# peaceminusones/Group-GAN-GCN-GAT

Hardware: AMD Instinct MI355X
Metric: scenes/sec (obs8/pred12, 20 peds) at 1/2/4/8 GPUs; ADE/FDE vs ref (higher is better)
Workload: dtype fp32; 1 GPU; train iteration = D-step + G-step (best_k=20, Adam), GAT generator; BASELINE configs[1] shape (batch 64); scenes_per_gpu=64, global_batch=64, obs_len=8, pred_len=12, generator=gat, hip_graph=True, parallelism=dp1

## Files before the change

### group-gan-gcn-gat_amd/csrc/glue.hip

```cpp
#include "sgg_common.h"

namespace sgg {

namespace {

__global__ void __launch_bounds__(256) traj_cat_kernel(const float* __restrict__ head, int ldh, int T0,
                                                       const float* __restrict__ a, int lda,
                                                       const float* __restrict__ b, int ldb, int T1, int B,
                                                       float* __restrict__ out, const float* __restrict__ pos0,
                                                       float* __restrict__ start) {
  const int NB = b ? 2 * B : B;
  const int total = (T0 + T1) * NB;
  for (int e = blockIdx.x * blockDim.x + threadIdx.x; e < total + (start ? NB : 0); e += gridDim.x * blockDim.x) {
    if (e >= total) {
      const int p = e - total;
      reinterpret_cast<float2*>(start)[p] = reinterpret_cast<const float2*>(pos0)[p < B ? p : p - B];
      continue;
    }
    const int t = e / NB, p = e - t * NB;
    const float* src;
    if (t < T0) {
      src = head + (size_t)t * ldh + 2 * (p < B ? p : p - B);
    } else if (p < B) {
      src = a + (size_t)(t - T0) * lda + 2 * p;
// ... 8 lines not shown
                                                           const float* __restrict__ z, int nz,
                                                           const int64_t* __restrict__ best, int first_k,
                                                           int copies, const int32_t* __restrict__ ped_scene,
                                                           int S, int B, const float* __restrict__ last_rel,
                                                           float* __restrict__ h0, float* __restrict__ rel0) {
  const int D = Dc + nz;
  const int total = copies * B * D;
  for (int e = blockIdx.x * blockDim.x + threadIdx.x; e < total; e += gridDim.x * blockDim.x) {
    const int row = e / D, c = e - row * D;
    const int r = row / B, p = row - r * B;
    float v;
    if (c < Dc) {
      v = ctx[(size_t)p * ldc + c];
    } else {
      const int s = ped_scene[p];
      const int k = (best && r == 0) ? (int)best[s] : first_k + r - (best ? 1 : 0);
      v = z[((size_t)k * S + s) * nz + (c - Dc)];
    }
    h0[e] = v;
    if (c < 2) rel0[(size_t)row * 2 + c] = last_rel[(size_t)p * 2 + c];
  }
}

constexpr int kL2MaxElems = SGG_POOL_MAX_PEDS * 32;

__device__ __forceinline__ void stage_mask(float* msk, const float* __restrict__ mask, int ldm, int o, int n, int T,
                                           int t0, int nt) {
  for (int e = t0; e < n * T; e += nt) {
    const int i = e / T, t = e - i * T;
    msk[e] = mask[(size_t)(o + i) * ldm + t];
  }
}

__global__ void __launch_bounds__(512) l2_select_kernel(const float* __restrict__ pred, const float* __restrict__ gt,
                                                        const float* __restrict__ mask, int ldm,
                                                        const int32_t* __restrict__ scene_off, int T, int B, int k,
                                                        int64_t* __restrict__ best) {
  __shared__ float part[256];
  __shared__ float msk[kL2MaxElems];
  const int s = blockIdx.x;
  const int o = scene_off[s], n = scene_off[s + 1] - o;
  const int lane = threadIdx.x & 63, wave = threadIdx.x >> 6;
  const float2* g2 = reinterpret_cast<const float2*>(gt);
  const float2* p2 = reinterpret_cast<const float2*>(pred);
  const int tot = n * T;
  const bool staged = tot <= kL2MaxElems;
  if (staged) stage_mask(msk, mask, ldm, o, n, T, threadIdx.x, blockDim.x);
  __syncthreads();
  constexpr int kRS = 4;
  for (int r0 = wave; r0 < k; r0 += 8 * kRS) {
    float acc[kRS];
#pragma unroll
    for (int j = 0; j < kRS; ++j) acc[j] = 0.f;
    for (int e0 = lane; e0 < tot; e0 += 256) {
      float mk[4];
      float2 g[4], q[kRS][4];
#pragma unroll
      for (int u = 0; u < 4; ++u) {
        const int e = min(e0 + 64 * u, tot - 1);
        const int t = e / n, i = e - t * n, p = o + i;
        mk[u] = staged ? msk[i * T + t] : mask[(size_t)p * ldm + t];
        g[u] = g2[(size_t)t * B + p];
#pragma unroll
        for (int j = 0; j < kRS; ++j) {
          const int r = min(r0 + 8 * j, k - 1);
          q[j][u] = p2[((size_t)t * k + r) * B + p];
        }
      }
#pragma unroll
      for (int j = 0; j < kRS; ++j)
#pragma unroll
        for (int u = 0; u < 4; ++u)
          if (e0 + 64 * u < tot) {
            const float dx = g[u].x - q[j][u].x, dy = g[u].y - q[j][u].y;
            acc[j] = fmaf(mk[u], fmaf(dx, dx, dy * dy), acc[j]);
          }
    }
#pragma unroll
    for (int j = 0; j < kRS; ++j) {
      const float a = wave_sum(acc[j]);
      if (lane == 0 && r0 + 8 * j < k) part[r0 + 8 * j] = a;
    }
  }
  __syncthreads();
  if (threadIdx.x == 0) {
    int bi = 0;
    float bv = part[0];
    for (int r = 1; r < k; ++r)
      if (part[r] < bv) {
        bv = part[r];
        bi = r;
      }
    best[s] = bi;
  }
}

__device__ __forceinline__ void l2_scene(const float* __restrict__ pred, int ldp, const float2* __restrict__ g2,
                                         const float* __restrict__ mask, int ldm, int o, int n, int T, int B,
                                         float* msk, int lane, float& acc_out, float& ms_out) {
  const int tot = n * T;
  const bool staged = tot <= kL2MaxElems;
  if (staged) stage_mask(msk, mask, ldm, o, n, T, lane, 64);
  __builtin_amdgcn_fence(__ATOMIC_RELEASE, "wavefront");
  __builtin_amdgcn_wave_barrier();
  __builtin_amdgcn_fence(__ATOMIC_ACQUIRE, "wavefront");
  float acc = 0.f, ms = 0.f;
  for (int e0 = lane; e0 < tot; e0 += 256) {
    float mk[4];
    float2 g[4], q[4];
#pragma unroll
    for (int u = 0; u < 4; ++u) {
      const int e = min(e0 + 64 * u, tot - 1);
      const int t = e / n, i = e - t * n, p = o + i;
      mk[u] = staged ? msk[i * T + t] : mask[(size_t)p * ldm + t];
      g[u] = g2[(size_t)t * B + p];
      q[u] = *reinterpret_cast<const float2*>(pred + (size_t)t * ldp + 2 * p);
    }
// ... 99 lines not shown
  hipLaunchKernelGGL(traj_cat_kernel, dim3(grid_for(total, 256)), dim3(256), 0, (hipStream_t)stream, head, ldh, T0, a,
                     lda, b, ldb, T1, B, out, pos0, start);
  SGG_RETURN_LAUNCH("sgg_traj_cat");
}

extern "C" int sgg_decoder_init(const float* ctx, int ldc, int Dc, const float* z, int nz, const int64_t* best,
                                int first_k, int copies, const int32_t* ped_scene, int S, int B,
                                const float* last_rel, float* h0, float* rel0, void* stream) {
  SGG_CHECK_ARG(ctx && ped_scene && last_rel && h0 && rel0 && (nz == 0 || z), "sgg_decoder_init: null pointer");
  SGG_CHECK_ARG(Dc > 0 && nz >= 0 && ldc >= Dc && copies >= 1 && S >= 0 && B >= 0 && Dc + nz >= 2,
                "sgg_decoder_init: bad sizes");
  const long long total = (long long)copies * B * (Dc + nz);
  if (total == 0) return 0;
  hipLaunchKernelGGL(decoder_init_kernel, dim3(grid_for(total, 256)), dim3(256), 0, (hipStream_t)stream, ctx, ldc, Dc,
                     z, nz, best, first_k, copies, ped_scene, S, B, last_rel, h0, rel0);
  SGG_RETURN_LAUNCH("sgg_decoder_init");
}

extern "C" int sgg_l2_select(const float* pred, const float* gt, const float* mask, int ldm, const int32_t* scene_off,
                             int S, int T, int B, int k, int64_t* best, void* stream) {
  SGG_CHECK_ARG(pred && gt && mask && scene_off && best, "sgg_l2_select: null pointer");
  SGG_CHECK_ARG(S >= 0 && T >= 1 && B >= 0 && k >= 1 && k <= 256 && ldm >= T, "sgg_l2_select: bad sizes");
  if (S == 0) return 0;
  hipLaunchKernelGGL(l2_select_kernel, dim3(S), dim3(512), 0, (hipStream_t)stream, pred, gt, mask, ldm, scene_off, T,
                     B, k, best);
  SGG_RETURN_LAUNCH("sgg_l2_select");
}

extern "C" int sgg_l2_loss_fwd(const float* pred, int ldp, const float* gt, const float* mask, int ldm,
                               const int32_t* scene_off, int S, int T, int B, float w, float* loss, float* msum,
                               float* term_ws, void* stream) {
  SGG_CHECK_ARG(pred && gt && mask && scene_off && loss && msum && term_ws, "sgg_l2_loss_fwd: null pointer");
  SGG_CHECK_ARG(S >= 0 && T >= 1 && B >= 0 && ldm >= T && ldp >= 2 * B, "sgg_l2_loss_fwd: bad sizes");
  if (S > 0)
    hipLaunchKernelGGL(l2_terms_kernel, dim3(S), dim3(64), 0, (hipStream_t)stream, pred, ldp, gt, mask, ldm, scene_off,
                     T, B, w, msum, term_ws);
  hipLaunchKernelGGL(l2_sum_kernel, dim3(1), dim3(64), 0, (hipStream_t)stream, term_ws, S, loss);
  SGG_RETURN_LAUNCH("sgg_l2_loss_fwd");
}

extern "C" int sgg_l2_loss_bwd(const float* pred, int ldp, const float* gt, const float* mask, int ldm,
                               const int32_t* ped_scene, const float* msum, int T, int B, float w, const float* gout,
                               float* dpred, int ldd, void* stream) {
  SGG_CHECK_ARG(pred && gt && mask && ped_scene && msum && gout && dpred, "sgg_l2_loss_bwd: null pointer");
  SGG_CHECK_ARG(T >= 1 && B >= 0 && ldm >= T && ldp >= 2 * B && ldd >= 2 * B, "sgg_l2_loss_bwd: bad sizes");
  if (B == 0) return 0;
  hipLaunchKernelGGL(l2_loss_bwd_kernel, dim3(grid_for((long long)T * B, 256)), dim3(256), 0, (hipStream_t)stream,
                     pred, ldp, gt, mask, ldm, ped_scene, msum, T, B, w, gout, dpred, ldd);
// ... 15 lines not shown
```

### group-gan-gcn-gat_amd/csrc/grad.hip

```cpp
#include <string.h>

#include "sgg_common.h"

namespace sgg {

namespace {

constexpr int kRedJobs = SGG_RED_MAX + 2 * SGG_FOLDB_MAX;

struct FinishArgs {
  SggRed red[kRedJobs];
  unsigned char vec[kRedJobs];
  int nred;
  int blk0[kRedJobs + 1];
  SggL2Job l2[SGG_LOSSJOB_MAX];
  SggBceJob bce[SGG_LOSSJOB_MAX];
  int nl2, nbce;
};

__device__ __forceinline__ float phase_sum(const float* __restrict__ src, int rows, int ld, int col, int ph) {
  float s = 0.f;
  int r = ph;
  for (; r + 48 < rows; r += 64) {
    const float v0 = src[(size_t)r * ld + col], v1 = src[(size_t)(r + 16) * ld + col];
    const float v2 = src[(size_t)(r + 32) * ld + col], v3 = src[(size_t)(r + 48) * ld + col];
    s += v0;
    s += v1;
    s += v2;
    s += v3;
  }
  for (; r < rows; r += 16) s += src[(size_t)r * ld + col];
  return s;
}

__device__ __forceinline__ floatx4 phase_sum4(const float* __restrict__ src, int rows, int ld, int col, int ph) {
  floatx4 s = {0.f, 0.f, 0.f, 0.f};
  int r = ph;
  for (; r + 48 < rows; r += 64) {
    const floatx4 v0 = *reinterpret_cast<const floatx4*>(src + (size_t)r * ld + col);
    const floatx4 v1 = *reinterpret_cast<const floatx4*>(src + (size_t)(r + 16) * ld + col);
// ... 130 lines not shown
  for (int j = 0; j < SGG_LOSSJOB_MAX; ++j)
    if (j < a.nbce) bce_load(a.bce[j], in[j]);
  float ad[SGG_LOSSJOB_MAX];
#pragma unroll
  for (int j = 0; j < SGG_LOSSJOB_MAX; ++j) {
    ad[j] = 0.f;
    if (j < a.nbce && a.bce[j].total) {
      bool fromL2 = false;
      for (int k = 0; k < a.nl2; ++k) fromL2 |= a.bce[j].addend == a.l2[k].loss;
      if (!fromL2) ad[j] = *a.bce[j].addend;
    }
  }
  for (int k = 0; k < a.nl2; ++k) l2_value(a.l2[k], lv + k);
#pragma unroll
  for (int j = 0; j < SGG_LOSSJOB_MAX; ++j)
    if (j < a.nbce) {
      float addend = ad[j];
      for (int k = 0; k < a.nl2; ++k)
        if (a.bce[j].total && a.bce[j].addend == a.l2[k].loss) addend = lv[k];
      bce_value(a.bce[j], in[j], addend, reinterpret_cast<float(*)[kLossThreads / 64]>(&rpart[0][0]));
    }
}

__global__ void __launch_bounds__(1024) grad_finish_kernel(FinishArgs a) {
  __shared__ __attribute__((aligned(16))) float rpart[16][256];
  const int lw = a.nl2 + a.nbce > 0;
  const int b = (int)blockIdx.x - lw;
  if (b < 0) {
    loss_workgroup(a, rpart);
    return;
  }
  int j = 0;
  while (j + 1 < a.nred && b >= a.blk0[j + 1]) ++j;
  red_job(a.red[j], a.vec[j] != 0, b - a.blk0[j], rpart);
}

}

}

using namespace sgg;

extern "C" int sgg_grad_finish(const SggRed* reds, int nred, const SggFoldBwd* folds, int nfold, float* scratch,
                               size_t scratch_bytes, void* stream) {
  return sgg_grad_finish_losses(reds, nred, folds, nfold, scratch, scratch_bytes, nullptr, 0, nullptr, 0, stream);
}

extern "C" int sgg_grad_finish_losses(const SggRed* reds, int nred, const SggFoldBwd* folds, int nfold,
                                      float* scratch, size_t scratch_bytes, const SggL2Job* l2, int nl2,
                                      const SggBceJob* bce, int nbce, void* stream) {
  SGG_CHECK_ARG(nl2 >= 0 && nl2 <= SGG_LOSSJOB_MAX && nbce >= 0 && nbce <= SGG_LOSSJOB_MAX &&
                    (nl2 == 0 || l2) && (nbce == 0 || bce),
                "sgg_grad_finish_losses: 0 <= nl2, nbce <= %d (got %d, %d)", SGG_LOSSJOB_MAX, nl2, nbce);
  for (int j = 0; j < nl2; ++j) {
    const SggL2Job& d = l2[j];
    SGG_CHECK_ARG(d.loss && (d.S == 0 || d.term) && d.S >= 0, "sgg_grad_finish_losses: bad L2 job %d", j);
  }
  for (int j = 0; j < nbce; ++j) {
    const SggBceJob& d = bce[j];
    SGG_CHECK_ARG(d.ya && d.yb && d.loss && (d.n == 0 || d.x) && (!d.total || d.addend),
                  "sgg_grad_finish_losses: null pointer in BCE job %d", j);
    SGG_CHECK_ARG(d.n >= 0 && d.split >= 0 && d.split <= d.n, "sgg_grad_finish_losses: BCE job %d: bad sizes", j);
  }
  SGG_CHECK_ARG(nred >= 0 && nred <= SGG_RED_MAX && nfold >= 0 && nfold <= SGG_FOLDB_MAX,
                "sgg_grad_finish: 0 <= nred <= %d, 0 <= nfold <= %d (got %d, %d)", SGG_RED_MAX, SGG_FOLDB_MAX, nred,
                nfold);
  SGG_CHECK_ARG((nred == 0 || reds) && (nfold == 0 || (folds && scratch)), "sgg_grad_finish: null job list or scratch");
  FinishArgs a;
  memset(&a, 0, sizeof(a));
  int nj = 0;
  auto add_red = [&](const SggRed& d) {
    a.red[nj] = d;
    ++nj;
// ... 19 lines not shown
    SGG_CHECK_ARG(d.R >= 1 && d.R <= 512 && d.E >= 1 && d.E <= 128 && d.ldw >= d.E && d.lddw >= d.E,
                  "sgg_grad_finish: bad fold sizes in job %d (R %d E %d)", k, d.R, d.E);
    SGG_CHECK_ARG(d.dA_rows >= 0 && d.db_rows >= 0 && d.dA_col0 >= 0 && d.db_col0 >= 0 &&
                      d.dA_ld >= d.dA_col0 + 2 * d.R && d.db_ld >= d.db_col0 + d.R,
                  "sgg_grad_finish: bad (dA, dbias) sources in fold job %d", k);
    add_red(SggRed{d.dA_src, d.dA_rows, d.dA_ld, d.dA_col0, 2 * d.R, g, 0, 0, 0, 0});
    add_red(SggRed{d.db_src, d.db_rows, d.db_ld, d.db_col0, d.R, g + 2 * d.R, 0, 0, 0, 0});
    g += 3 * (size_t)d.R;
  }
  a.nred = nj;
  int blk = 0;
  for (int j = 0; j < nj; ++j) {
    const SggRed& d = a.red[j];
    a.vec[j] = d.ld % 4 == 0 && d.col0 % 4 == 0 && (reinterpret_cast<uintptr_t>(d.src) & 15) == 0;
    a.blk0[j] = blk;
    blk += a.vec[j] ? (d.cols + 255) / 256 : (d.cols + 63) / 64;
  }
  a.blk0[nj] = blk;
  for (int j = 0; j < nl2; ++j) a.l2[j] = l2[j];
  for (int j = 0; j < nbce; ++j) a.bce[j] = bce[j];
  a.nl2 = nl2;
  a.nbce = nbce;
  if (nl2 + nbce > 0) ++blk;
  hipStream_t st = (hipStream_t)stream;
  if (blk > 0) hipLaunchKernelGGL(grad_finish_kernel, dim3(blk), dim3(1024), 0, st, a);
  if (nfold > 0) {
    SggFoldBwd f[SGG_FOLDB_MAX];
    g = scratch;
    for (int k = 0; k < nfold; ++k) {
      f[k] = folds[k];
      f[k].dA_src = g;
      f[k].db_src = g + 2 * folds[k].R;
      g += 3 * (size_t)folds[k].R;
    }
    fold_bwd_multi(f, nfold, st);
  }
  SGG_RETURN_LAUNCH("sgg_grad_finish");
}
```

### group-gan-gcn-gat_amd/sgan/_native.py

```python
import ctypes
import os

import torch

from ._srchash import source_hash

_LIB_EXPLICIT = bool(os.environ.get("SGG_LIB"))
_LIB_PATH = os.environ.get("SGG_LIB") or os.path.join(os.path.dirname(os.path.abspath(__file__)), "_lib", "libsgg.so")

_i = ctypes.c_int
_f = ctypes.c_float
_p = ctypes.c_void_p
_sz = ctypes.c_size_t

MAX_HEADS = 4


class GatEncWeights(ctypes.Structure):
    _fields_ = [("Wi", _p * MAX_HEADS), ("ai", _p * MAX_HEADS), ("Wio", _p), ("aio", _p),
                ("Wg", _p * MAX_HEADS), ("ag", _p * MAX_HEADS), ("Wgo", _p), ("ago", _p), ("Woe", _p), ("boe", _p)]


class GatEncArgs(ctypes.Structure):
    _fields_ = [("X", _p), ("ldx", _i), ("labels", _p), ("scene_off", _p), ("S", _i), ("np", _i), ("nh", _i),
# ... 58 lines not shown
class TrajOut(ctypes.Structure):
    _fields_ = [("out", _p), ("NB", _i), ("T0", _i), ("col0", _i), ("ncol", _i), ("head", _p), ("ldh", _i),
                ("b", _p), ("ldb", _i), ("pos0", _p), ("start", _p)]


class PoolBatch(ctypes.Structure):
    _fields_ = [("U", _p), ("pos", _p), ("scene_off", _p), ("chunks", _p), ("nchunks", _i), ("max_rows", _i),
                ("gpw", _i), ("B", _i), ("max_n", _i), ("out", _p), ("argmax", _p), ("nchunks_dev", _p)]


class GatLayerSet(ctypes.Structure):
    _fields_ = [("x1", _p), ("ld1", _i), ("K1", _i), ("x2", _p), ("ld2", _i), ("K2", _i), ("seg_off", _p),
                ("nseg", _i), ("n", _i), ("max_seg", _i), ("xn", _p), ("rstd", _p), ("wh", _p), ("hp", _p), ("y", _p),
                ("ldy", _i)]


class L2Job(ctypes.Structure):
    _fields_ = [("term", _p), ("S", _i), ("loss", _p)]


class BceJob(ctypes.Structure):
    _fields_ = [("x", _p), ("n", _i), ("split", _i), ("ya", _p), ("yb", _p), ("w", _f), ("loss", _p),
                ("addend", _p), ("total", _p), ("nvalid", _p)]


SIGNATURES = {
    "sgg_version": (_i, []),
    "sgg_last_error": (ctypes.c_char_p, []),
    "sgg_source_hash": (ctypes.c_char_p, []),
    "sgg_xw": (_i, [_p, _i, _p, _i, _p, _i, _i, _p, _p, _i, _i, _i, _i, _i, _p]),
    "sgg_xw_bf16": (_i, [_p, _i, _p, _i, _p, _i, _i, _p, _p, _i, _i, _i, _i, _i, _p]),
    "sgg_pool_plan": (_i, [_p, _i, _i, _i, _i, _p, _i, _p, _p]),
    "sgg_pool_fwd": (_i, [_p, _p, _p, _p, _p, _p, _p, _i, _i, _i, _i, _i, _i, _p, _p, _p, _p]),
    "sgg_pool_plan_bf16": (_i, [_p, _i, _i, _i, _p, _i, _p, _p]),
    "sgg_pool_fwd_bf16": (_i, [_p, _p, _p, _p, _p, _p, _p, _i, _i, _i, _i, _i, _i, _p, _p, _p, _p]),
    "sgg_pool_fwd2": (_i, [ctypes.POINTER(PoolBatch), ctypes.POINTER(PoolBatch), _p, _p, _p, _i, _i, _p]),
    "sgg_pool_bwd_grid": (_i, [_i]),
    "sgg_pool_dh_dw": (_i, [_p, _i, _p, _i, _p, _i, _i, _p, _i, _i, _i, _p, _sz, _p]),
    "sgg_pool_bwd": (_i, [_p, _p, _p, _p, _p, _p, _p, _p, _i, _i, _i, _i, _p, _p, _p]),
    "sgg_gat_fwd": (_i, [_p, _i, _p, _p, _p, _p, _i, _i, _i, _f, _i, _i, _i, _p, _p, _i, _p]),
    "sgg_gat_bwd": (_i, [_p, _i, _p, _p, _p, _i, _i, _i, _f, _i, _i, _i, _p, _p, _p, _i, _p, _p, _p, _p]),
    "sgg_gat_fwd_ex": (_i, [_p, _i, _p, _p, _p, _p, _p, _i, _i, _i, _f, _i, _i, _i, _p, _p, _i, _p]),
    "sgg_gat_bwd_ex": (_i, [_p, _i, _p, _p, _p, _p, _i, _i, _i, _f, _i, _i, _i, _p, _p, _p, _i, _p, _p, _p, _p, _p,
                            _p]),
    "sgg_gat_bwd_ex_work_bytes": (_sz, [_i, _i, _i]),
    "sgg_gat_layer_lds_bytes": (_sz, [_i, _i, _i]),
# ... 11 lines not shown
    "sgg_lstm_bwd_split": (_i, [_p, _p, _p, _p, _p, _p, _p, _p, _p, _p, _i, _i, _i, _i, _p, _p, _p, _p, _p]),
    "sgg_lstm_bwd_tail": (_i, [_p, _p, _p, _p, _p, _p, _p, _i, _i, _i, _i, _p, _p]),
    "sgg_lstm_fwd_seg": (_i, [_sargs, _i, _p]),
    "sgg_lstm_fwd_seg2": (_i, [_sargs, _i, _sargs, _i, _p]),
    "sgg_lstm_fwd_seg3": (_i, [_sargs, _i, _sargs, _i, _sargs, _i, _p]),
    "sgg_lstm_bwd_shared": (_i, [_p, _p, _p, _p, _p, _p, _p, _i, _i, _i, _i, _i, _p, _p, _p]),
    "sgg_lstm_u_ok": (_i, [_i, _i, _i, _i, _i, _i]),
    "sgg_lstm_fwd_u": (_i, [_p, _p, _p, _p, _p, _p, _i, _i, _i, _p, _p, _p, _p, _i, _p, _i, _p, _p]),
    "sgg_head_ok": (_i, [_i, _i]),
    "sgg_head_slab_cols": (_i, [_i, _i]),
    "sgg_head_fwd": (_i, [_p, _i, _i, _i, _i, _p, _p, _p, _p, _i, _p, _p, _p]),
    "sgg_head_bwd": (_i, [_p, _i, _i, _i, _i, _p, _p, _p, _p, _p, _i, _p, _i, _p, _p, _p, _p, _i, _f, _p, _p]),
    "sgg_head_fwdbwd": (_i, [_p, _i, _i, _i, _i, _p, _p, _p, _p, _i, _p, _p, _i, _p, _p, _p, _p, _i, _f, _p, _p]),
    "sgg_xtw_partial": (_i, [_p, _i, _p, _i, _p, _i, _i, _i, _i, _i, _p, _sz, _p]),
    "sgg_grad_finish": (_i, [ctypes.POINTER(Red), _i, ctypes.POINTER(FoldBwd), _i, _p, _sz, _p]),
    "sgg_lstm_fwd_dec": (_i, [ctypes.POINTER(DecInit), _p, _p, _p, _p, _p, _i, _i, _i, _p, _p, _p, _p, _p,
                              ctypes.POINTER(TrajOut), _p]),
    "sgg_lstm_fwd_dec2": (_i, [ctypes.POINTER(DecInit), ctypes.POINTER(DecInit), _p, _p, _p, _p, _p, _i, _i, _i, _i,
                               _p, _p, ctypes.POINTER(TrajOut), _p]),
    "sgg_lstm_fwd_dec_seg": (_i, [ctypes.POINTER(DecInit), _p, _p, _p, _p, _p, _i, _i, _i, _p, _p, _p, _p, _p,
                                  ctypes.POINTER(TrajOut), _sargs, _i, _p]),
    "sgg_grad_finish_losses": (_i, [ctypes.POINTER(Red), _i, ctypes.POINTER(FoldBwd), _i, _p, _sz,
                                    ctypes.POINTER(L2Job), _i, ctypes.POINTER(BceJob), _i, _p]),
    "sgg_adam_parts": (_i, [ctypes.c_longlong]),
    "sgg_adam_step": (_i, [_p, _p, _p, _p, _p, _i, ctypes.c_double, ctypes.c_double, ctypes.c_double, _f, _f, _p, _p,
                          _sz, _p]),
    "sgg_xtw": (_i, [_p, _i, _p, _i, _p, _i, _i, _i, _i, _p, _i, _i, _p, _p, _sz, _p]),
    "sgg_fold_fwd": (_i, [_p, _i, _i, _i, _p, _p, _p, _p, _p, _p, _p]),
    "sgg_fold_fwd_multi": (_i, [ctypes.POINTER(Fold), _i, _p]),
    "sgg_fold_bwd": (_i, [_p, _i, _i, _i, _p, _p, _p, _p, _p, _i, _p, _p, _p, _p]),
    "sgg_lstm_fwd": (_i, [_p, _p, _p, _p, _p, _p, _p, _p, _i, _i, _i, _i, _p, _p, _p, _p, _p]),
    "sgg_lstm_state_floats": (ctypes.c_longlong, [_i, _i, _i, _i]),
    "sgg_lstm_wpart_rows": (_i, [_i, _i]),
    "sgg_lstm_kernel_name": (ctypes.c_char_p, [_i, _i, _i, _i, _i]),
    "sgg_lstm_bwd": (_i, [_p, _p, _p, _p, _p, _p, _p, _p, _p, _p, _i, _i, _i, _i, _p, _p, _p, _p, _p, _p]),
    "sgg_bce_fwd": (_i, [_p, _i, _i, _p, _p, _f, _p, _p, _p, _p, _p]),
    "sgg_bce_bwd": (_i, [_p, _i, _i, _p, _p, _f, _p, _p, _p, _p]),
    "sgg_gatenc_param_size": (_i, [_i]),
    "sgg_gatenc_lds_bytes": (ctypes.c_longlong, [_i, _i, _i]),
    "sgg_gatenc_saved_floats": (ctypes.c_longlong, [_i, _i, _i]),
    "sgg_gatenc_fwd": (_i, [_pargs, _p]),
    "sgg_gatenc_fwd2": (_i, [_pargs, _pargs, _p]),
    "sgg_gatenc_bwd": (_i, [_pargs, _p]),
    "sgg_gcnmod_param_size": (_i, [_i, _i]),
    "sgg_gcnmod_slab_rows": (_i, [_i]),
    "sgg_gcnmod_lds_bytes": (ctypes.c_longlong, [_i, _i, _i, _i]),
# ... 67 lines not shown
```

### group-gan-gcn-gat_amd/sgan/kernels.py

```python
import contextlib
import functools
import os
import weakref

import torch

from . import _native as N

GATENC_FUSED = os.environ.get("SGG_GATENC_FUSED", "1") != "0"
GATENC_SAVE = os.environ.get("SGG_GATENC_SAVE", "1") != "0"
DUAL_POOL_BWD = os.environ.get("SGG_DUAL_POOL_BWD", "1") != "0"
SIDE_STREAM = os.environ.get("SGG_SIDE_STREAM", "0") == "1"


DEBUG = os.environ.get("SGG_DEBUG", "0") == "1"


def _lib():
    return N.load()


def _req(t, name, dtype=torch.float32):
    if not t.is_cuda:
        raise N.NativeError("%s must be a device tensor (no CPU path)" % name)
# ... 334 lines not shown

def _queue_loss(kind, job, keep, outs):
    _LOSS[kind].append(job)
    _LOSS["keep"] += [t.untyped_storage() for t in keep if t is not None]
    _LOSS["out"].update(t.data_ptr() for t in outs)


def _loss_pending(t):
    return t is not None and t.data_ptr() in _LOSS["out"]


def _take_losses():
    l2, bce, keep = _LOSS["l2"], _LOSS["bce"], _LOSS["keep"]
    _LOSS.update(l2=[], bce=[], keep=[], out=set())
    return l2, bce, keep


def flush_losses():
    l2, bce, keep = _take_losses()
    if l2 or bce:
        _finish_launch([], [], keep, l2, bce)


@contextlib.contextmanager
def defer_grad_finish():
    if os.environ.get("SGG_CHECK_DEFER") == "1":
        yield
        return
    _DEFER[0] += 1
    try:
        yield
    finally:
        _DEFER[0] -= 1
        if _DEFER[0] == 0:
            grad_flush()


def grad_flush():
    if not _PENDING:
        flush_losses()
    while _PENDING:
        reds, folds, keep = [], [], []
        while _PENDING and len(reds) + len(_PENDING[0].reds) <= N.RED_MAX \
                and len(folds) + len(_PENDING[0].folds) <= N.FOLDB_MAX:
            gf = _PENDING.pop(0)
            reds += gf.reds
            folds += gf.folds
            keep += gf.keep
        if not reds and not folds:
            raise N.NativeError("grad_flush: a queued finish exceeds the job limits")
        l2, bce = [], []
        if not _PENDING:
            l2, bce, lkeep = _take_losses()
            keep = keep + lkeep
        _finish_launch(reds, folds, keep, l2, bce)


def _finish_launch(reds_l, folds_l, keep, l2_l=(), bce_l=()):
    lib = _lib()
    assert len(reds_l) <= N.RED_MAX and len(folds_l) <= N.FOLDB_MAX
    assert len(l2_l) <= N.LOSSJOB_MAX and len(bce_l) <= N.LOSSJOB_MAX
    reds = (N.Red * max(1, len(reds_l)))(*reds_l)
    folds = (N.FoldBwd * max(1, len(folds_l)))(*folds_l)
    l2 = (N.L2Job * max(1, len(l2_l)))(*l2_l)
    bce = (N.BceJob * max(1, len(bce_l)))(*bce_l)
    nr, nf, nl, nb = len(reds_l), len(folds_l), len(l2_l), len(bce_l)
    dev = keep[0].device
    scratch = torch.empty(max(1, sum(3 * f.R for f in folds_l)), device=dev, dtype=torch.float32)

    def launch(reds=reds, folds=folds, nr=nr, nf=nf, l2=l2, bce=bce, nl=nl, nb=nb, keep=list(keep)):
        N.check(lib.sgg_grad_finish_losses(reds, nr, folds, nf, N.ptr(scratch), scratch.numel() * 4, l2, nl, bce, nb,
                                           N.stream_ptr()), "sgg_grad_finish")
    launch()
    if timer.active:
        nb = sum(4.0 * r.rows * r.cols for r in reds_l) + sum(4.0 * 3 * f.R * max(f.dA_rows, f.db_rows)
                                                               for f in folds_l)
        timer.add("sgg::grad_finish_kernel", (nr, nf, tuple((r.rows, r.cols) for r in reds_l)), nb / 4.0, nb,
                  launch)


class _XW(torch.autograd.Function):
    @staticmethod
    def forward(ctx, x, w, bias, trans_w, act):
        y = xw_raw(x, w, bias, trans_w, act)
        ctx.trans_w, ctx.act, ctx.has_bias = trans_w, act, bias is not None
        ctx.save_for_backward(x, w, y if act else None)
        return y

    @staticmethod
    def backward(ctx, dy):
        x, w, y = ctx.saved_tensors
        dy = dy.contiguous()
        m = y if ctx.act else None
        dx = dw = db = None
        if ctx.needs_input_grad[0]:
            dx = xw_raw(dy, w, None, not ctx.trans_w, 0, mask=m, prec="fp32")
        if ctx.needs_input_grad[1] or (ctx.has_bias and ctx.needs_input_grad[2]):
            with side(x, dy, m):
                dw, cs = xtw(x, dy, colsum=True, trans_c=ctx.trans_w, mask=m)
            db = cs if ctx.has_bias else None
        return dx, dw, db, None, None
# ... 2168 lines not shown


class _DecoderInit(torch.autograd.Function):
    @staticmethod
    def forward(ctx, cvec, z, best, first_k, copies, scenes, last_rel, lazy):
        ctx.dy_link = getattr(cvec, "_sgg_copies_link", None)
        cvec = _rows(cvec, "ctx")
        B, Dc = cvec.shape
        nz = z.shape[-1] if z is not None else 0
        h0 = torch.empty(copies * B, Dc + nz, device=cvec.device, dtype=torch.float32)
        rel0 = torch.empty(copies * B, 2, device=cvec.device, dtype=torch.float32)
        zc = _req(z, "z").contiguous() if z is not None else None
        last = _req(last_rel, "last_rel").contiguous()
        if B != scenes.B or tuple(last.shape) != (B, 2):
            raise ValueError("decoder_init: context rows %d / last_rel %s vs the scenes' %d peds"
                             % (B, tuple(last.shape), scenes.B))
        if zc is not None:
            need_k = first_k + copies - (1 if best is not None else 0)
            if zc.dim() != 3 or zc.shape[1] != scenes.S or zc.shape[0] < max(need_k, 1):
                raise ValueError("decoder_init: noise %s must be (>= %d draws, %d scenes, nz)"
                                 % (tuple(zc.shape), need_k, scenes.S))
            if best is not None and (best.numel() != scenes.S or best.dtype != torch.int64):
                raise ValueError("decoder_init: best must be the %d scenes' int64 sample indices" % scenes.S)
        ps = scenes.ped_scene_i32()
        args = (N.ptr(cvec), cvec.stride(0), Dc, N.ptr(zc), nz, N.ptr(best), int(first_k), int(copies), N.ptr(ps),
                scenes.S, B, N.ptr(last), N.ptr(h0), N.ptr(rel0))

        keep = tuple(t.detach() for t in (cvec, zc, best, ps, last) if t is not None)

        def materialize(h0_buf, rel0_buf, keep=keep):
            N.check(_lib().sgg_decoder_init(*args[:-2], N.ptr(h0_buf), N.ptr(rel0_buf), N.stream_ptr()),
                    "sgg_decoder_init")
        if lazy:
            di = N.DecInit(N.ptr(cvec), cvec.stride(0), Dc, N.ptr(zc), nz, N.ptr(best), int(first_k), N.ptr(ps),
                           scenes.S, B, N.ptr(last))
            di._keep = keep
            h0._sgg_dinit = (di, keep, materialize)
        else:
            materialize(h0, rel0)
        ctx.dims = (copies, B, Dc)
        ctx.mark_non_differentiable(rel0)
        ctx.set_materialize_grads(False)
        return h0, rel0

    @staticmethod
    def backward(ctx, dh0, _drel0):
        copies, B, Dc = ctx.dims
        d = dh0.view(copies, B, -1)[:, :, :Dc]
        if copies > 1 and ctx.dy_link is not None and dh0.is_contiguous():
            ctx.dy_link.put(dh0, copies, B * dh0.shape[1], dh0.shape[1])
            return d[0], None, None, None, None, None, None, None
        return (d[0] if copies == 1 else d.sum(0)), None, None, None, None, None, None, None


def decoder_init(cvec, z, best, first_k, copies, scenes, last_rel, lazy=False):
    return _DecoderInit.apply(cvec, z, best, first_k, copies, scenes, last_rel, bool(lazy and DEC_INIT_FUSED))


def l2_select(pred, gt, mask, scenes, k):
    best = torch.empty(scenes.S, device=pred.device, dtype=torch.int64)
    pred = _req(pred, "pred").contiguous()
    N.check(_lib().sgg_l2_select(N.ptr(pred), N.ptr(_req(gt, "gt").contiguous()), N.ptr(mask), mask.stride(0),
                                 N.ptr(scenes.scene_off), scenes.S, gt.shape[0], scenes.B, int(k), N.ptr(best),
                                 N.stream_ptr()), "sgg_l2_select")
    return best


class _L2Loss(torch.autograd.Function):
    @staticmethod
    def forward(ctx, pred, gt, mask, scenes, w):
        _req(pred, "pred")
        assert pred.stride(1) == 2 and pred.stride(2) == 1 and mask.stride(1) == 1
        gt = _req(gt, "gt").contiguous()
        T, B = gt.shape[0], gt.shape[1]
        loss = torch.empty((), device=pred.device, dtype=torch.float32)
        term = None
        if _loss_deferrable("l2"):
            term = torch.empty(max(scenes.S, 1), device=pred.device, dtype=torch.float32)
            _queue_loss("l2", N.L2Job(N.ptr(term), scenes.S, N.ptr(loss)), (term, loss), (loss,))
            msum = None
        else:
            msum = torch.empty(scenes.S, device=pred.device, dtype=torch.float32)
            term = torch.empty(scenes.S, device=pred.device, dtype=torch.float32)
            N.check(_lib().sgg_l2_loss_fwd(N.ptr(pred), pred.stride(0), N.ptr(gt), N.ptr(mask), mask.stride(0),
                                           N.ptr(scenes.scene_off), scenes.S, T, B, float(w), N.ptr(loss),
                                           N.ptr(msum), N.ptr(term), N.stream_ptr()), "sgg_l2_loss_fwd")
        ctx.save_for_backward(pred, gt, mask, msum, term)
# ... 51 lines not shown
```

### group-gan-gcn-gat_amd/sgan/models.py

```python
import torch
import torch.nn as nn
import torch.nn.functional as F

from . import kernels as K
from .scene import SceneIndex

_SCENE_CACHE = {"sse": None, "ver": None, "dev": None, "idx": None}


def scene_index(seq_start_end, device):
    c = _SCENE_CACHE
    if c["sse"] is seq_start_end and c["ver"] == seq_start_end._version and c["dev"] == device:
        return c["idx"]
    idx = SceneIndex.from_seq_start_end(seq_start_end, device)
    c.update(sse=seq_start_end, ver=seq_start_end._version, dev=device, idx=idx)
    return idx


def _scenes(seq_start_end, device, scenes):
    if scenes is not None:
        return scenes
    return scene_index(seq_start_end, device)


# ... 609 lines not shown
            comp = K.GcnModCompanion(h_a.view(-1, H), g_a[-1], sc_a, x2=pool_a)
            module = self.gcn_module
        y_b = module((h_b.view(-1, H), pool_b), sse_b, obs_b[-1], g_b[-1], scenes=sc_b, link=link, companion=comp)
        return comp.y, y_b

    def decode(self, noise_input, obs_traj, obs_traj_rel, seq_start_end, user_noise=None, *, scenes=None,
               copies=1, noise_index=None):
        sc = _scenes(seq_start_end, obs_traj.device, scenes)
        if (not self.pool_every_timestep and self.noise_dim and self.noise_mix_type == "global"
                and user_noise is not None and self.num_layers == 1):
            nz = self.noise_first_dim
            if noise_index is None:
                z, best, first_k = user_noise.reshape(copies, sc.S, nz), None, 0
            else:
                (best, first_k), z = noise_index, user_noise
            z = z.to(noise_input.device, non_blocking=True)
            h0, rel0 = K.decoder_init(noise_input, z, best, first_k, copies, sc, obs_traj_rel[-1], lazy=True)
            with K.final_state_unused():
                _h, rel = K.lstm_sequence(rel0, self.decoder.decoder, self.decoder.spatial_embedding, h0=h0, c0=None,
                                          proj=self.decoder.hidden2pos, decoder=True, T=self.pred_len)
            return rel
        if noise_index is not None and user_noise is not None:
            best, first_k = noise_index
            zk = user_noise.to(noise_input.device)
            ar = torch.arange(sc.S, device=zk.device)
            parts = [zk[best, ar]] if best is not None else []
            parts += [zk[first_k + r] for r in range(copies - len(parts))]
            user_noise = torch.cat(parts, 0)
        last_pos, last_rel = obs_traj[-1], obs_traj_rel[-1]
        if copies > 1:
            if self.pool_every_timestep:
                raise NotImplementedError("decode(copies>1) with per-step pooling: run forward() per sample")
            sc = sc.repeat(copies)
            noise_input = noise_input.repeat(copies, 1)
            last_pos, last_rel = last_pos.repeat(copies, 1), last_rel.repeat(copies, 1)
            seq_start_end = None
        decoder_h = self.add_noise(noise_input, seq_start_end, user_noise=user_noise, scenes=sc).unsqueeze(0)
        decoder_c = (torch.zeros(self.num_layers, sc.B, self.decoder_h_dim, device=obs_traj.device)
                     if self.pool_every_timestep else None)
        out, _ = self.decoder(last_pos, last_rel, (decoder_h, decoder_c), seq_start_end, scenes=sc)
        return out


class TrajectoryDiscriminator(nn.Module):
    def __init__(self, obs_len, pred_len, embedding_dim=64, h_dim=64, mlp_dim=1024, num_layers=1,
                 activation="relu", batch_norm=True, dropout=0.0, d_type="local"):
# ... 37 lines not shown
```

### include/sgg.h

```cpp
#ifndef SGG_H
#define SGG_H

#include <stdint.h>
#include <stddef.h>

#ifdef __cplusplus
extern "C" {
#endif

#define SGG_E_ARG (-1)

int sgg_version(void);
const char* sgg_last_error(void);
const char* sgg_source_hash(void);

#define SGG_POOL_MAX_PEDS 64
#define SGG_GAT_MAX_NODES 128

int sgg_xw(const float* X, int ldx, const float* Xmask, int ldm, const float* W, int ldw, int trans_w,
           const float* bias, float* Y, int ldy, int M, int K, int N, int act, void* stream);

int sgg_xw_bf16(const float* X, int ldx, const float* Xmask, int ldm, const float* W, int ldw, int trans_w,
                const float* bias, float* Y, int ldy, int M, int K, int N, int act, void* stream);

// ... 141 lines not shown
                    size_t scratch_bytes, void* stream);

#define SGG_LOSSJOB_MAX 2
typedef struct {
  const float* term;
  int S;
  float* loss;
} SggL2Job;
typedef struct {
  const float* x;
  int n;
  int split;
  const float* ya;
  const float* yb;
  float w;
  float* loss;
  const float* addend;
  float* total;
  const int32_t* nvalid;
} SggBceJob;
int sgg_grad_finish_losses(const SggRed* reds, int nred, const SggFoldBwd* folds, int nfold, float* scratch,
                           size_t scratch_bytes, const SggL2Job* l2, int nl2, const SggBceJob* bce, int nbce,
                           void* stream);

int sgg_head_ok(int K, int N1);
int sgg_head_slab_cols(int K, int N1);
int sgg_head_fwd(const float* X, int ldx, int M, int K, int N1, const float* W1, const float* b1, const float* w2,
                 const float* b2, int act, float* hid, float* Y, void* stream);
int sgg_head_bwd(const float* X, int ldx, int M, int K, int N1, const float* W1, const float* w2, const float* hid,
                 const float* Y, const float* dY, int act, float* dX, int lddx, float* wslab, const float* bce_g,
                 const float* bce_ya, const float* bce_yb, int bce_split, float bce_w, const int32_t* bce_nvalid,
                 void* stream);
int sgg_head_fwdbwd(const float* X, int ldx, int M, int K, int N1, const float* W1, const float* b1, const float* w2,
                    const float* b2, int act, float* Y, float* dX, int lddx, float* wslab, const float* bce_g,
                    const float* bce_ya, const float* bce_yb, int bce_split, float bce_w, const int32_t* bce_nvalid,
                    void* stream);

int sgg_fold_fwd(const float* W, int ldw, int R, int E, const float* We, const float* be,
                 const float* b1, const float* b2, float* A, float* bias, void* stream);
#define SGG_FOLD_MAX 8
typedef struct {
  const float* W;
  int ldw;
  int R;
  int E;
  const float* We;
// ... 223 lines not shown
```

Before: 137,300 scenes/s.

## Fold best-of-k L2 argmin selection into the grad-finish kernel launch

The per-scene best-of-k L2 argmin kernel is deferred while inside a deferred grad-finish region. It then runs as extra workgroups of the grad_finish kernel, two scenes per 1024-thread block, with the masks staged in the existing reduction shared memory. This removes one kernel launch per iteration and lets the selection run alongside the gradient reductions. Consumers of best (decoder_init, add_noise) flush any held job first, which adds ordering bookkeeping and a risk of stale results if a consumer is missed.

```diff
diff --git a/group-gan-gcn-gat_amd/csrc/glue.hip b/group-gan-gcn-gat_amd/csrc/glue.hip
--- a/group-gan-gcn-gat_amd/csrc/glue.hip
+++ b/group-gan-gcn-gat_amd/csrc/glue.hip
@@ -1,4 +1,5 @@
 #include "sgg_common.h"
+#include "l2_body.h"
 
 namespace sgg {
 
@@ -54,77 +55,14 @@
   }
 }
 
-constexpr int kL2MaxElems = SGG_POOL_MAX_PEDS * 32;
-
-__device__ __forceinline__ void stage_mask(float* msk, const float* __restrict__ mask, int ldm, int o, int n, int T,
-                                           int t0, int nt) {
-  for (int e = t0; e < n * T; e += nt) {
-    const int i = e / T, t = e - i * T;
-    msk[e] = mask[(size_t)(o + i) * ldm + t];
-  }
-}
-
-__global__ void __launch_bounds__(512) l2_select_kernel(const float* __restrict__ pred, const float* __restrict__ gt,
-                                                        const float* __restrict__ mask, int ldm,
-                                                        const int32_t* __restrict__ scene_off, int T, int B, int k,
-                                                        int64_t* __restrict__ best) {
-  __shared__ float part[256];
+__global__ void __launch_bounds__(kL2SelThreads) l2_select_kernel(const float* __restrict__ pred,
+                                                                  const float* __restrict__ gt,
+                                                                  const float* __restrict__ mask, int ldm,
+                                                                  const int32_t* __restrict__ scene_off, int T, int B,
+                                                                  int k, int64_t* __restrict__ best) {
+  __shared__ float part[kL2SelMaxK];
   __shared__ float msk[kL2MaxElems];
-  const int s = blockIdx.x;
-  const int o = scene_off[s], n = scene_off[s + 1] - o;
-  const int lane = threadIdx.x & 63, wave = threadIdx.x >> 6;
-  const float2* g2 = reinterpret_cast<const float2*>(gt);
-  const float2* p2 = reinterpret_cast<const float2*>(pred);
-  const int tot = n * T;
-  const bool staged = tot <= kL2MaxElems;
-  if (staged) stage_mask(msk, mask, ldm, o, n, T, threadIdx.x, blockDim.x);
-  __syncthreads();
-  constexpr int kRS = 4;
-  for (int r0 = wave; r0 < k; r0 += 8 * kRS) {
-    float acc[kRS];
-#pragma unroll
-    for (int j = 0; j < kRS; ++j) acc[j] = 0.f;
-    for (int e0 = lane; e0 < tot; e0 += 256) {
-      float mk[4];
-      float2 g[4], q[kRS][4];
-#pragma unroll
-      for (int u = 0; u < 4; ++u) {
-        const int e = min(e0 + 64 * u, tot - 1);
-        const int t = e / n, i = e - t * n, p = o + i;
-        mk[u] = staged ? msk[i * T + t] : mask[(size_t)p * ldm + t];
-        g[u] = g2[(size_t)t * B + p];
-#pragma unroll
-        for (int j = 0; j < kRS; ++j) {
-          const int r = min(r0 + 8 * j, k - 1);
-          q[j][u] = p2[((size_t)t * k + r) * B + p];
-        }
-      }
-#pragma unroll
-      for (int j = 0; j < kRS; ++j)
-#pragma unroll
-        for (int u = 0; u < 4; ++u)
-          if (e0 + 64 * u < tot) {
-            const float dx = g[u].x - q[j][u].x, dy = g[u].y - q[j][u].y;
-            acc[j] = fmaf(mk[u], fmaf(dx, dx, dy * dy), acc[j]);
-          }
-    }
-#pragma unroll
-    for (int j = 0; j < kRS; ++j) {
-      const float a = wave_sum(acc[j]);
-      if (lane == 0 && r0 + 8 * j < k) part[r0 + 8 * j] = a;
-    }
-  }
-  __syncthreads();
-  if (threadIdx.x == 0) {
-    int bi = 0;
-    float bv = part[0];
-    for (int r = 1; r < k; ++r)
-      if (part[r] < bv) {
-        bv = part[r];
-        bi = r;
-      }
-    best[s] = bi;
-  }
+  l2_select_scene(pred, gt, mask, ldm, scene_off, T, B, k, best, blockIdx.x, threadIdx.x, true, part, msk);
 }
 
 __device__ __forceinline__ void l2_scene(const float* __restrict__ pred, int ldp, const float2* __restrict__ g2,
@@ -270,8 +208,8 @@
   SGG_CHECK_ARG(pred && gt && mask && scene_off && best, "sgg_l2_select: null pointer");
   SGG_CHECK_ARG(S >= 0 && T >= 1 && B >= 0 && k >= 1 && k <= 256 && ldm >= T, "sgg_l2_select: bad sizes");
   if (S == 0) return 0;
-  hipLaunchKernelGGL(l2_select_kernel, dim3(S), dim3(512), 0, (hipStream_t)stream, pred, gt, mask, ldm, scene_off, T,
-                     B, k, best);
+  hipLaunchKernelGGL(l2_select_kernel, dim3(S), dim3(kL2SelThreads), 0, (hipStream_t)stream, pred, gt, mask, ldm,
+                     scene_off, T, B, k, best);
   SGG_RETURN_LAUNCH("sgg_l2_select");
 }
 
diff --git a/group-gan-gcn-gat_amd/csrc/grad.hip b/group-gan-gcn-gat_amd/csrc/grad.hip
--- a/group-gan-gcn-gat_amd/csrc/grad.hip
+++ b/group-gan-gcn-gat_amd/csrc/grad.hip
@@ -1,6 +1,7 @@
 #include <string.h>
 
 #include "sgg_common.h"
+#include "l2_body.h"
 
 namespace sgg {
 
@@ -16,6 +17,8 @@
   SggL2Job l2[SGG_LOSSJOB_MAX];
   SggBceJob bce[SGG_LOSSJOB_MAX];
   int nl2, nbce;
+  SggL2SelJob sel;
+  int nsel;
 };
 
 __device__ __forceinline__ float phase_sum(const float* __restrict__ src, int rows, int ld, int col, int ph) {
@@ -192,14 +195,28 @@
     }
 }
 
+static_assert(2 * kL2MaxElems <= 16 * 256, "the two scenes' mask blocks are staged in rpart");
+__device__ void select_workgroup(const SggL2SelJob& d, int b, float (*rpart)[256]) {
+  __shared__ float part[2][kL2SelMaxK];
+  const int half = threadIdx.x / kL2SelThreads, tid = threadIdx.x - half * kL2SelThreads;
+  const int s = 2 * b + half;
+  l2_select_scene(d.pred, d.gt, d.mask, d.ldm, d.scene_off, d.T, d.B, d.k, d.best, s, tid, s < d.S, part[half],
+                  &rpart[0][0] + half * kL2MaxElems);
+}
+
 __global__ void __launch_bounds__(1024) grad_finish_kernel(FinishArgs a) {
   __shared__ __attribute__((aligned(16))) float rpart[16][256];
   const int lw = a.nl2 + a.nbce > 0;
-  const int b = (int)blockIdx.x - lw;
+  int b = (int)blockIdx.x - lw;
   if (b < 0) {
     loss_workgroup(a, rpart);
     return;
   }
+  if (b < a.nsel) {
+    select_workgroup(a.sel, b, rpart);
+    return;
+  }
+  b -= a.nsel;
   int j = 0;
   while (j + 1 < a.nred && b >= a.blk0[j + 1]) ++j;
   red_job(a.red[j], a.vec[j] != 0, b - a.blk0[j], rpart);
@@ -213,12 +230,25 @@
 
 extern "C" int sgg_grad_finish(const SggRed* reds, int nred, const SggFoldBwd* folds, int nfold, float* scratch,
                                size_t scratch_bytes, void* stream) {
-  return sgg_grad_finish_losses(reds, nred, folds, nfold, scratch, scratch_bytes, nullptr, 0, nullptr, 0, stream);
+  return sgg_grad_finish_sel(reds, nred, folds, nfold, scratch, scratch_bytes, nullptr, 0, nullptr, 0, nullptr, stream);
 }
 
 extern "C" int sgg_grad_finish_losses(const SggRed* reds, int nred, const SggFoldBwd* folds, int nfold,
                                       float* scratch, size_t scratch_bytes, const SggL2Job* l2, int nl2,
                                       const SggBceJob* bce, int nbce, void* stream) {
+  return sgg_grad_finish_sel(reds, nred, folds, nfold, scratch, scratch_bytes, l2, nl2, bce, nbce, nullptr, stream);
+}
+
+extern "C" int sgg_grad_finish_sel(const SggRed* reds, int nred, const SggFoldBwd* folds, int nfold, float* scratch,
+                                   size_t scratch_bytes, const SggL2Job* l2, int nl2, const SggBceJob* bce, int nbce,
+                                   const SggL2SelJob* sel, void* stream) {
+  if (sel) {
+    SGG_CHECK_ARG(sel->pred && sel->gt && sel->mask && sel->scene_off && sel->best,
+                  "sgg_grad_finish_sel: null pointer in the argmin job");
+    SGG_CHECK_ARG(sel->S >= 0 && sel->T >= 1 && sel->B >= 0 && sel->k >= 1 && sel->k <= kL2SelMaxK &&
+                      sel->ldm >= sel->T,
+                  "sgg_grad_finish_sel: bad sizes in the argmin job");
+  }
   SGG_CHECK_ARG(nl2 >= 0 && nl2 <= SGG_LOSSJOB_MAX && nbce >= 0 && nbce <= SGG_LOSSJOB_MAX &&
                     (nl2 == 0 || l2) && (nbce == 0 || bce),
                 "sgg_grad_finish_losses: 0 <= nl2, nbce <= %d (got %d, %d)", SGG_LOSSJOB_MAX, nl2, nbce);
@@ -284,6 +314,11 @@
   a.nl2 = nl2;
   a.nbce = nbce;
   if (nl2 + nbce > 0) ++blk;
+  if (sel && sel->S > 0) {
+    a.sel = *sel;
+    a.nsel = (sel->S + 1) / 2;
+    blk += a.nsel;
+  }
   hipStream_t st = (hipStream_t)stream;
   if (blk > 0) hipLaunchKernelGGL(grad_finish_kernel, dim3(blk), dim3(1024), 0, st, a);
   if (nfold > 0) {
diff --git a/group-gan-gcn-gat_amd/csrc/l2_body.h b/group-gan-gcn-gat_amd/csrc/l2_body.h
--- /dev/null
+++ b/group-gan-gcn-gat_amd/csrc/l2_body.h
@@ -0,0 +1,79 @@
+#pragma once
+#include "sgg_common.h"
+
+namespace sgg {
+
+constexpr int kL2MaxElems = SGG_POOL_MAX_PEDS * 32;
+constexpr int kL2SelThreads = 512;
+constexpr int kL2SelMaxK = 256;
+
+__device__ __forceinline__ void stage_mask(float* msk, const float* __restrict__ mask, int ldm, int o, int n, int T,
+                                           int t0, int nt) {
+  for (int e = t0; e < n * T; e += nt) {
+    const int i = e / T, t = e - i * T;
+    msk[e] = mask[(size_t)(o + i) * ldm + t];
+  }
+}
+
+__device__ __forceinline__ void l2_select_scene(const float* __restrict__ pred, const float* __restrict__ gt,
+                                                const float* __restrict__ mask, int ldm,
+                                                const int32_t* __restrict__ scene_off, int T, int B, int k,
+                                                int64_t* __restrict__ best, int s, int tid, bool live, float* part,
+                                                float* msk) {
+  const int o = live ? scene_off[s] : 0, n = live ? scene_off[s + 1] - o : 0;
+  const int lane = tid & 63, wave = tid >> 6;
+  const float2* g2 = reinterpret_cast<const float2*>(gt);
+  const float2* p2 = reinterpret_cast<const float2*>(pred);
+  const int tot = n * T;
+  const bool staged = tot <= kL2MaxElems;
+  if (live && staged) stage_mask(msk, mask, ldm, o, n, T, tid, kL2SelThreads);
+  __syncthreads();
+  constexpr int kRS = 4;
+  for (int r0 = wave; live && r0 < k; r0 += 8 * kRS) {
+    float acc[kRS];
+#pragma unroll
+    for (int j = 0; j < kRS; ++j) acc[j] = 0.f;
+    for (int e0 = lane; e0 < tot; e0 += 256) {
+      float mk[4];
+      float2 g[4], q[kRS][4];
+#pragma unroll
+      for (int u = 0; u < 4; ++u) {
+        const int e = min(e0 + 64 * u, tot - 1);
+        const int t = e / n, i = e - t * n, p = o + i;
+        mk[u] = staged ? msk[i * T + t] : mask[(size_t)p * ldm + t];
+        g[u] = g2[(size_t)t * B + p];
+#pragma unroll
+        for (int j = 0; j < kRS; ++j) {
+          const int r = min(r0 + 8 * j, k - 1);
+          q[j][u] = p2[((size_t)t * k + r) * B + p];
+        }
+      }
+#pragma unroll
+      for (int j = 0; j < kRS; ++j)
+#pragma unroll
+        for (int u = 0; u < 4; ++u)
+          if (e0 + 64 * u < tot) {
+            const float dx = g[u].x - q[j][u].x, dy = g[u].y - q[j][u].y;
+            acc[j] = fmaf(mk[u], fmaf(dx, dx, dy * dy), acc[j]);
+          }
+    }
+#pragma unroll
+    for (int j = 0; j < kRS; ++j) {
+      const float a = wave_sum(acc[j]);
+      if (lane == 0 && r0 + 8 * j < k) part[r0 + 8 * j] = a;
+    }
+  }
+  __syncthreads();
+  if (live && tid == 0) {
+    int bi = 0;
+    float bv = part[0];
+    for (int r = 1; r < k; ++r)
+      if (part[r] < bv) {
+        bv = part[r];
+        bi = r;
+      }
+    best[s] = bi;
+  }
+}
+
+}
diff --git a/group-gan-gcn-gat_amd/sgan/_native.py b/group-gan-gcn-gat_amd/sgan/_native.py
--- a/group-gan-gcn-gat_amd/sgan/_native.py
+++ b/group-gan-gcn-gat_amd/sgan/_native.py
@@ -104,6 +104,11 @@
 class BceJob(ctypes.Structure):
     _fields_ = [("x", _p), ("n", _i), ("split", _i), ("ya", _p), ("yb", _p), ("w", _f), ("loss", _p),
                 ("addend", _p), ("total", _p), ("nvalid", _p)]
+
+
+class L2SelJob(ctypes.Structure):
+    _fields_ = [("pred", _p), ("gt", _p), ("mask", _p), ("ldm", _i), ("scene_off", _p), ("S", _i), ("T", _i),
+                ("B", _i), ("k", _i), ("best", _p)]
 
 
 SIGNATURES = {
@@ -161,6 +166,8 @@
                                   ctypes.POINTER(TrajOut), _sargs, _i, _p]),
     "sgg_grad_finish_losses": (_i, [ctypes.POINTER(Red), _i, ctypes.POINTER(FoldBwd), _i, _p, _sz,
                                     ctypes.POINTER(L2Job), _i, ctypes.POINTER(BceJob), _i, _p]),
+    "sgg_grad_finish_sel": (_i, [ctypes.POINTER(Red), _i, ctypes.POINTER(FoldBwd), _i, _p, _sz,
+                                 ctypes.POINTER(L2Job), _i, ctypes.POINTER(BceJob), _i, ctypes.POINTER(L2SelJob), _p]),
     "sgg_adam_parts": (_i, [ctypes.c_longlong]),
     "sgg_adam_step": (_i, [_p, _p, _p, _p, _p, _i, ctypes.c_double, ctypes.c_double, ctypes.c_double, _f, _f, _p, _p,
                           _sz, _p]),
diff --git a/group-gan-gcn-gat_amd/sgan/kernels.py b/group-gan-gcn-gat_amd/sgan/kernels.py
--- a/group-gan-gcn-gat_amd/sgan/kernels.py
+++ b/group-gan-gcn-gat_amd/sgan/kernels.py
@@ -1,4 +1,5 @@
 import contextlib
+import ctypes
 import functools
 import os
 import weakref
@@ -380,6 +381,24 @@
         _finish_launch([], [], keep, l2, bce)
 
 
+L2_RIDE = os.environ.get("SGG_L2_RIDE", "1") != "0"
+_L2SEL = [None]
+
+
+def _take_l2_select():
+    held, _L2SEL[0] = _L2SEL[0], None
+    return held
+
+
+def flush_l2_select():
+    held = _take_l2_select()
+    if held is not None:
+        job, keep, launch, work = held
+        launch()
+        if timer.active:
+            timer.add("sgg::l2_select_kernel", (job.S, job.T, job.B, job.k), work[0], work[1], launch)
+
+
 @contextlib.contextmanager
 def defer_grad_finish():
     if os.environ.get("SGG_CHECK_DEFER") == "1":
@@ -391,7 +410,10 @@
     finally:
         _DEFER[0] -= 1
         if _DEFER[0] == 0:
-            grad_flush()
+            try:
+                grad_flush()
+            finally:
+                flush_l2_select()
 
 
 def grad_flush():
@@ -425,16 +447,22 @@
     nr, nf, nl, nb = len(reds_l), len(folds_l), len(l2_l), len(bce_l)
     dev = keep[0].device
     scratch = torch.empty(max(1, sum(3 * f.R for f in folds_l)), device=dev, dtype=torch.float32)
-
-    def launch(reds=reds, folds=folds, nr=nr, nf=nf, l2=l2, bce=bce, nl=nl, nb=nb, keep=list(keep)):
-        N.check(lib.sgg_grad_finish_losses(reds, nr, folds, nf, N.ptr(scratch), scratch.numel() * 4, l2, nl, bce, nb,
-                                           N.stream_ptr()), "sgg_grad_finish")
+    held = _take_l2_select()
+    sel, skeep, swork = (held[0], held[1], held[3]) if held is not None else (None, (), (0.0, 0.0))
+
+    def launch(reds=reds, folds=folds, nr=nr, nf=nf, l2=l2, bce=bce, nl=nl, nb=nb, keep=list(keep) + list(skeep),
+               sel=sel):
+        N.check(lib.sgg_grad_finish_sel(reds, nr, folds, nf, N.ptr(scratch), scratch.numel() * 4, l2, nl, bce, nb,
+                                        ctypes.byref(sel) if sel is not None else None, N.stream_ptr()),
+                "sgg_grad_finish")
     launch()
     if timer.active:
         nb = sum(4.0 * r.rows * r.cols for r in reds_l) + sum(4.0 * 3 * f.R * max(f.dA_rows, f.db_rows)
                                                                for f in folds_l)
-        timer.add("sgg::grad_finish_kernel", (nr, nf, tuple((r.rows, r.cols) for r in reds_l)), nb / 4.0, nb,
-                  launch)
+        key = (nr, nf, tuple((r.rows, r.cols) for r in reds_l))
+        if sel is not None:
+            key += (("l2_select", sel.S, sel.k),)
+        timer.add("sgg::grad_finish_kernel", key, nb / 4.0 + swork[0], nb + swork[1], launch)
 
 
 class _XW(torch.autograd.Function):
@@ -2649,6 +2677,8 @@
                                  % (tuple(zc.shape), need_k, scenes.S))
             if best is not None and (best.numel() != scenes.S or best.dtype != torch.int64):
                 raise ValueError("decoder_init: best must be the %d scenes' int64 sample indices" % scenes.S)
+        if best is not None:
+            flush_l2_select()
         ps = scenes.ped_scene_i32()
         args = (N.ptr(cvec), cvec.stride(0), Dc, N.ptr(zc), nz, N.ptr(best), int(first_k), int(copies), N.ptr(ps),
                 scenes.S, B, N.ptr(last), N.ptr(h0), N.ptr(rel0))
@@ -2687,9 +2717,22 @@
 def l2_select(pred, gt, mask, scenes, k):
     best = torch.empty(scenes.S, device=pred.device, dtype=torch.int64)
     pred = _req(pred, "pred").contiguous()
-    N.check(_lib().sgg_l2_select(N.ptr(pred), N.ptr(_req(gt, "gt").contiguous()), N.ptr(mask), mask.stride(0),
-                                 N.ptr(scenes.scene_off), scenes.S, gt.shape[0], scenes.B, int(k), N.ptr(best),
-                                 N.stream_ptr()), "sgg_l2_select")
+    gt = _req(gt, "gt").contiguous()
+    off, S, T, B, k = scenes.scene_off, scenes.S, gt.shape[0], scenes.B, int(k)
+    lib = _lib()
+
+    def launch():
+        N.check(lib.sgg_l2_select(N.ptr(pred), N.ptr(gt), N.ptr(mask), mask.stride(0), N.ptr(off), S, T, B, k,
+                                  N.ptr(best), N.stream_ptr()), "sgg_l2_select")
+    work = (6.0 * T * B * k, 4.0 * (2 * T * B * k + 2 * T * B + T * B) + 8.0 * S)
+    if L2_RIDE and _DEFER[0] > 0 and S > 0:
+        flush_l2_select()
+        job = N.L2SelJob(N.ptr(pred), N.ptr(gt), N.ptr(mask), mask.stride(0), N.ptr(off), S, T, B, k, N.ptr(best))
+        _L2SEL[0] = (job, [t.untyped_storage() for t in (pred, gt, mask, off, best)], launch, work)
+        return best
+    launch()
+    if timer.active:
+        timer.add("sgg::l2_select_kernel", (S, T, B, k), work[0], work[1], launch)
     return best
 
 
diff --git a/group-gan-gcn-gat_amd/sgan/models.py b/group-gan-gcn-gat_amd/sgan/models.py
--- a/group-gan-gcn-gat_amd/sgan/models.py
+++ b/group-gan-gcn-gat_amd/sgan/models.py
@@ -655,6 +655,8 @@
             return rel
         if noise_index is not None and user_noise is not None:
             best, first_k = noise_index
+            if best is not None:
+                K.flush_l2_select()
             zk = user_noise.to(noise_input.device)
             ar = torch.arange(sc.S, device=zk.device)
             parts = [zk[best, ar]] if best is not None else []
diff --git a/include/sgg.h b/include/sgg.h
--- a/include/sgg.h
+++ b/include/sgg.h
@@ -187,6 +187,22 @@
 int sgg_grad_finish_losses(const SggRed* reds, int nred, const SggFoldBwd* folds, int nfold, float* scratch,
                            size_t scratch_bytes, const SggL2Job* l2, int nl2, const SggBceJob* bce, int nbce,
                            void* stream);
+
+typedef struct {
+  const float* pred;
+  const float* gt;
+  const float* mask;
+  int ldm;
+  const int32_t* scene_off;
+  int S;
+  int T;
+  int B;
+  int k;
+  int64_t* best;
+} SggL2SelJob;
+int sgg_grad_finish_sel(const SggRed* reds, int nred, const SggFoldBwd* folds, int nfold, float* scratch,
+                        size_t scratch_bytes, const SggL2Job* l2, int nl2, const SggBceJob* bce, int nbce,
+                        const SggL2SelJob* sel, void* stream);
 
 int sgg_head_ok(int K, int N1);
 int sgg_head_slab_cols(int K, int N1);
```

Measured after the change: 138,400 scenes/s (median of 2 runs). No clear change (+0.8%).
